# gusanagy/Hybrid-Diffusion-Underwater-Atmopheric-Image-Enhancement

Measured on AMD Instinct MI355X. Metric: denoising-steps/sec (256x256, T=1000), higher is better.
Workload: dtype f32 (tensors and accumulation fp32; every operand of the attention contractions as 2xfp16 pieces -- scores: a balance per product term, four terms at d_head 16 / three at d_head 32; P.V: three terms -- and of the 3x3 convs behind GroupNorm likewise (other 3x3 convs: 3xbf16 pieces), on the 16-bit MFM

## Files before the change

### hybrid-diffusion-underwater-atmopheric-image-enhancement_amd/csrc/attention_x3p.hip

```cpp
#include <stdlib.h>

#include "common.h"
#include "device.h"

using namespace hdiff;

namespace {

constexpr int D = 32;
constexpr int KT = 64;
constexpr int THREADS = 256;
constexpr int NQT = 3;

__global__ __launch_bounds__(THREADS, 2) void mha_flash_fwd_x3p_kernel(const __bf16* __restrict__ ws, float* __restrict__ out,
                                                                      float* __restrict__ lse2, int C, int L, float one) {
  constexpr int KS = D / 16;
  constexpr int KROWB = D * 2 + 16;
  constexpr int KPART = KT * KROWB;
  constexpr int VROWB = KT * 2 + 8;
  constexpr int VPART = D * VROWB;
  constexpr int NKC = NQT * KT * D / 8;
  constexpr int NVC = 2 * D * 8;
  constexpr int NLD = (NKC + NVC) / THREADS;
  static_assert((NKC + NVC) % THREADS == 0, "staging geometry");
  constexpr int QB = 256;
  constexpr int VBASE = NQT * KPART;
  constexpr int BUFB = (VBASE + 2 * VPART + 15) / 16 * 16;
  __shared__ __attribute__((aligned(16))) unsigned char smem[2][BUFB];

  const int tid = threadIdx.x, lane = tid & 63, wave = tid >> 6;
  const int l31 = lane & 31, h = lane >> 5;
  const TileId tile = xcd_tile();
  const int head = tile.head, b = tile.b;
  const int heads = gridDim.y;
  const int qblk0 = tile.x * QB + wave * 64;
  const size_t piece = (size_t)L * D;
  const __bf16* qs = ws + ((size_t)b * heads + head) * F_COUNT * piece;
  const __bf16* ks = qs + F_K * piece;
  const __bf16* vs = qs + F_V * piece;
  const int ntiles = L / KT;

  u32x4 qop[2][NQT][KS];
#pragma unroll
  for (int G = 0; G < 2; ++G) {
    const int q = qblk0 + 32 * G + l31;
#pragma unroll
    for (int p = 0; p < 2; ++p)
#pragma unroll
      for (int s = 0; s < KS; ++s)
        qop[G][p][s] = *reinterpret_cast<const u32x4*>(qs + p * piece + (size_t)q * D + 16 * s + 8 * h);
    const unsigned dn2 = PAIR_DOWN2;
#pragma unroll
    for (int s = 0; s < KS; ++s) {
      unsigned w4[4];
#pragma unroll
      for (int w = 0; w < 4; ++w) asm("v_pk_mul_f16 %0, %1, %2" : "=v"(w4[w]) : "v"(qop[G][0][s][w]), "v"(dn2));
      qop[G][2][s] = u32x4{w4[0], w4[1], w4[2], w4[3]};
    }
  }

  const unsigned char* gsrc[NLD];
  int lds_off[NLD];
  int gstep[NLD];
#pragma unroll
  for (int i = 0; i < NLD; ++i) {
    const int c = i * THREADS + tid;
    if (c < NKC) {
      const int p = c / (KT * D / 8), rem = c - p * (KT * D / 8);
      const int key = rem / (D / 8), part = rem - key * (D / 8);
      gsrc[i] = reinterpret_cast<const unsigned char*>(ks + p * piece) + (size_t)rem * 16;
      lds_off[i] = p * KPART + key * KROWB + part * 16;
      gstep[i] = KT * D * 2;
    } else {
      const int cv = c - NKC;
      const int p = cv / (D * 8), rem = cv - p * (D * 8);
      const int d = rem >> 3, seg = rem & 7;
      gsrc[i] = reinterpret_cast<const unsigned char*>(vs + p * piece + (size_t)d * L) + seg * 16;
      lds_off[i] = VBASE + p * VPART + d * VROWB + seg * 16;
      gstep[i] = KT * 2;
    }
  }
  u32x4 stage[NLD];
  auto stage_load = [&](int t) {
#pragma unroll
    for (int i = 0; i < NLD; ++i) stage[i] = *reinterpret_cast<const u32x4*>(gsrc[i] + (size_t)t * gstep[i]);
  };
  auto stage_store = [&](int buf) {
#pragma unroll
    for (int i = 0; i < NLD; ++i) {
      unsigned char* dst = &smem[buf][lds_off[i]];
      *reinterpret_cast<u32x2*>(dst) = u32x2{stage[i][0], stage[i][1]};
      *reinterpret_cast<u32x2*>(dst + 8) = u32x2{stage[i][2], stage[i][3]};
    }
  };

  const int kaddr = l31 * KROWB + 16 * h;
  int vaddr[2];
#pragma unroll
  for (int p = 0; p < 2; ++p) vaddr[p] = p * VPART + l31 * VROWB + 8 * h;

  f32x16 O[2], negm16;
  f32x2 l_run[2];
  float negm2[2] = {0.f, 0.f};
#pragma unroll
  for (int G = 0; G < 2; ++G) {
    l_run[G] = f32x2{0.f, 0.f};
#pragma unroll
    for (int r = 0; r < 16; ++r) O[G][r] = 0.f;
  }
#pragma unroll
  for (int r = 0; r < 16; ++r) negm16[r] = 0.f;

  auto load_k = [&](int buf, int kb, u32x4 (&kop)[NQT][KS]) {
    const unsigned char* kbuf = smem[buf] + kb * 32 * KROWB + kaddr;
#pragma unroll
    for (int p = 0; p < NQT; ++p)
#pragma unroll
      for (int s = 0; s < KS; ++s) kop[p][s] = *reinterpret_cast<const u32x4*>(kbuf + p * KPART + 32 * s);
  };
  auto load_v = [&](int buf, int kb, u32x4 (&vop)[2][2]) {
    const unsigned char* vbuf = smem[buf] + VBASE + kb * 64;
#pragma unroll
    for (int ab = 0; ab < 2; ++ab)
#pragma unroll
      for (int p = 0; p < 2; ++p) {
        const unsigned char* src = vbuf + vaddr[p] + 32 * ab;
        const u32x2 lo = *reinterpret_cast<const u32x2*>(src);
        const u32x2 hi2 = *reinterpret_cast<const u32x2*>(src + 16);
        vop[ab][p] = u32x4{lo[0], lo[1], hi2[0], hi2[1]};
      }
  };
  auto qk = [&](const u32x4 (&kop)[NQT][KS], int G, f32x16 c) {
    f32x16 S = c;
#pragma unroll
    for (int term = 0; term < NQT; ++term)
#pragma unroll
      for (int s = 0; s < KS; ++s) {
        u32x4 qb = qop[G][term][s];
        if ((HDIFF_MUTANT & 2) && term == 1)
#pragma unroll
          for (int w = 0; w < 4; ++w) qb[w] &= 0xffe0ffe0u;
        S = mfma_f16(kop[term][s], qb, S);
      }
    return S;
  };
  auto exp_pairs = [&](const f32x16& S, u32x4 (&pop)[2][2], float& sum0, float& sum1) {
    sum0 = 0.f; sum1 = 0.f;
#pragma unroll
    for (int j = 0; j < 4; ++j) {
      const float p0 = __builtin_amdgcn_exp2f(S[4 * j]), p1 = __builtin_amdgcn_exp2f(S[4 * j + 1]);
      const float p2 = __builtin_amdgcn_exp2f(S[4 * j + 2]), p3 = __builtin_amdgcn_exp2f(S[4 * j + 3]);
      sum0 += p0 + p2;
      sum1 += p1 + p3;
      unsigned a0, a1, c0, c1;
      split2(p0, p1, one, a0, a1);
      split2(p2, p3, one, c0, c1);
      const int ab = j >> 1, o = (j & 1) * 2;
      pop[ab][0][o] = a0; pop[ab][1][o] = a1;
      pop[ab][0][o + 1] = c0; pop[ab][1][o + 1] = c1;
    }
  };
  auto softmax_pairs = [&](f32x16& S, int G, u32x4 (&pop)[2][2]) {
    float sum0, sum1;
    exp_pairs(S, pop, sum0, sum1);
    if (__builtin_amdgcn_ballot_w64(sum0 + sum1 >= P_TRIP) != 0ull) {
      float mx = fmaxf(fmaxf(S[0], S[1]), fmaxf(S[2], S[3]));
#pragma unroll
      for (int j = 1; j < 4; ++j) mx = fmaxf(mx, fmaxf(fmaxf(S[4 * j], S[4 * j + 1]), fmaxf(S[4 * j + 2], S[4 * j + 3])));
      mx = fmaxf(mx, __shfl_xor(mx, 32, 64));
      const float delta = (mx > P_SHIFT + 1.0f) ? __builtin_ceilf(mx - P_SHIFT) : 0.f;
      const int e = -(int)delta;
#pragma unroll
      for (int r = 0; r < 16; ++r) O[G][r] = __builtin_ldexpf(O[G][r], e);
      l_run[G][0] = __builtin_ldexpf(l_run[G][0], e);
      l_run[G][1] = __builtin_ldexpf(l_run[G][1], e);
      negm2[G] -= delta;
#pragma unroll
      for (int r = 0; r < 16; ++r) S[r] -= delta;
      exp_pairs(S, pop, sum0, sum1);
    }
    l_run[G][0] += sum0;
    l_run[G][1] += sum1;
  };
  auto pv = [&](const u32x4 (&vop)[2][2], const u32x4 (&pop)[2][2], int G) {
#pragma unroll
    for (int ab = 0; ab < 2; ++ab) {
      O[G] = mfma_f16(vop[ab][1], pop[ab][0], O[G]);
      O[G] = mfma_f16(vop[ab][0], pop[ab][1], O[G]);
      O[G] = mfma_f16(vop[ab][0], pop[ab][0], O[G]);
    }
  };

  stage_load(0);
  stage_store(0);
  __syncthreads();
  stage_load(ntiles > 1 ? 1 : 0);
  {
    u32x4 K0[NQT][KS];
    load_k(0, 0, K0);
    const f32x16 s0 = qk(K0, 0, negm16), s1 = qk(K0, 1, negm16);
    float t0 = s0[0], t1 = s1[0];
#pragma unroll
    for (int r = 1; r < 16; ++r) { t0 = fmaxf(t0, s0[r]); t1 = fmaxf(t1, s1[r]); }
    negm2[0] = P_SHIFT - fmaxf(t0, __shfl_xor(t0, 32, 64));
    negm2[1] = P_SHIFT - fmaxf(t1, __shfl_xor(t1, 32, 64));
  }
  auto block = [&](int buf, int kb) {
    u32x4 kop[NQT][KS], vop[2][2];
    load_k(buf, kb, kop);
    load_v(buf, kb, vop);
    f32x16 S2[2];
#pragma unroll
    for (int G = 0; G < 2; ++G) {
      float nm = negm2[G];
      asm volatile("" : "+v"(nm));
#pragma unroll
      for (int r = 0; r < 16; ++r) negm16[r] = nm;
      S2[G] = qk(kop, G, negm16);
    }
#pragma unroll
    for (int G = 0; G < 2; ++G) {
      u32x4 pop[2][2];
      softmax_pairs(S2[G], G, pop);
      pv(vop, pop, G);
    }
  };
  block(0, 0);
  block(0, 1);
  stage_store(1);
  __syncthreads();
  for (int t = 1; t < ntiles; ++t) {
    const int buf = t & 1;
    stage_load((t + 1 < ntiles) ? t + 1 : t);
    block(buf, 0);
    block(buf, 1);
    stage_store(buf ^ 1);
    __syncthreads();
  }

  float* obase = out + ((size_t)b * C + (size_t)head * D) * L;
  const float* vinv = reinterpret_cast<const float*>(qs + 8 * piece);
#pragma unroll
  for (int G = 0; G < 2; ++G) {
    float lt = l_run[G][0] + l_run[G][1];
    lt += __shfl_xor(lt, 32, 64);
    const bool bad = !(lt < OVERFLOW_LIMIT);
    const float inv = bad ? __builtin_nanf("") : 1.0f / lt;
    const int q = qblk0 + 32 * G + l31;
    if (lse2 != nullptr && h == 0)
      lse2[((size_t)b * heads + head) * L + q] = bad ? __builtin_nanf("") : __builtin_amdgcn_logf(lt) - negm2[G];
#pragma unroll
    for (int r = 0; r < 16; ++r) {
      const int d = 8 * (r >> 2) + 4 * h + (r & 3);
      obase[(size_t)d * L + q] = (O[G][r] * inv) * vinv[d];
    }
  }
}

}

namespace hdiff {

int64_t mha_fwd_x3p_workspace(int B, int C, int heads, int L) {
  const int Dh = C / heads;
  if ((Dh != 16 && Dh != 32) || L % 256 != 0 || L < 512) return 0;
  return (int64_t)B * C * L * F_COUNT * 2 + mha_fwd_h2_tail_bytes(B, C);
}

void launch_mha_fwd_x3p(const float* qkv, float* o, float* lse2, int B, int C, int heads, int L, float qscale, void* ws,
                        hipStream_t stream) {
  launch_qk_split_h2(qkv, ws, B, C, heads, L, qscale, stream);
  launch_v_split_h2(qkv, ws, B, C, heads, L, stream);
  hipLaunchKernelGGL(mha_flash_fwd_x3p_kernel, dim3(L / 256, heads, B), dim3(THREADS), 0, stream, (const __bf16*)ws, o, lse2, C, L, 1.0f);
}

}
```

Baseline: 3.045.

## Move rare softmax rescale into out-of-line asm subsection and keep per-group negm vectors

The rarely taken online-softmax rescale path (max reduction, O/l rescale, re-exponentiation) moves into inline-asm blocks placed in a cold subsection behind a scalar branch, so the hot path stays straight-line and the compiler does not keep registers live for it. The running max offset is now held as two persistent 16-wide accumulator-init vectors that are pinned to fixed VGPR ranges, so they no longer need to be broadcast before each QK MFMA. A sched_barrier also separates successive blocks. The hand-written asm and hard-coded register tuples (v[0:15], v[32:47]) are fragile and can clash with the compiler's register allocation. It also relies on manually inserted s_nop hazard padding.

```diff
diff --git a/hybrid-diffusion-underwater-atmopheric-image-enhancement_amd/csrc/attention_x3p.hip b/hybrid-diffusion-underwater-atmopheric-image-enhancement_amd/csrc/attention_x3p.hip
--- a/hybrid-diffusion-underwater-atmopheric-image-enhancement_amd/csrc/attention_x3p.hip
+++ b/hybrid-diffusion-underwater-atmopheric-image-enhancement_amd/csrc/attention_x3p.hip
@@ -11,6 +11,128 @@
 constexpr int KT = 64;
 constexpr int THREADS = 256;
 constexpr int NQT = 3;
+
+#define X3P_RARE_BEGIN "s_cmp_lg_u64 %[cond], 0\n\ts_cbranch_scc1 .Lx3pr_%=\n.Lx3pb_%=:\n\t.subsection 1\n.Lx3pr_%=:\n\t"
+#define X3P_RARE_END "s_branch .Lx3pb_%=\n\t.subsection 0"
+
+__device__ __forceinline__ float x3p_rare_delta(unsigned long long cond, const f32x16& S, int bp32) {
+  float delta, t, u;
+  asm volatile(X3P_RARE_BEGIN
+               "v_max3_f32 %[t], %[s0], %[s1], %[s2]\n\t"
+               "v_max3_f32 %[u], %[s3], %[s4], %[s5]\n\t"
+               "v_max3_f32 %[t], %[t], %[s6], %[s7]\n\t"
+               "v_max3_f32 %[u], %[u], %[s8], %[s9]\n\t"
+               "v_max3_f32 %[t], %[t], %[s10], %[s11]\n\t"
+               "v_max3_f32 %[u], %[u], %[s12], %[s13]\n\t"
+               "v_max3_f32 %[t], %[t], %[s14], %[s15]\n\t"
+               "v_max_f32 %[t], %[t], %[u]\n\t"
+               "s_nop 1\n\t"
+               "ds_bpermute_b32 %[u], %[bp32], %[t]\n\t"
+               "s_waitcnt lgkmcnt(0)\n\t"
+               "v_max_f32 %[t], %[t], %[u]\n\t"
+               "v_subrev_f32 %[u], 8.0, %[t]\n\t"
+               "v_ceil_f32 %[u], %[u]\n\t"
+               "v_cmp_lt_f32 vcc, 0x41100000, %[t]\n\t"
+               "v_cndmask_b32 %[d], 0, %[u], vcc\n\t"
+               X3P_RARE_END
+               : [d] "=&v"(delta), [t] "=&v"(t), [u] "=&v"(u)
+               : [cond] "s"(cond), [bp32] "v"(bp32), [s0] "v"(S[0]), [s1] "v"(S[1]), [s2] "v"(S[2]), [s3] "v"(S[3]), [s4] "v"(S[4]),
+                 [s5] "v"(S[5]), [s6] "v"(S[6]), [s7] "v"(S[7]), [s8] "v"(S[8]), [s9] "v"(S[9]), [s10] "v"(S[10]), [s11] "v"(S[11]),
+                 [s12] "v"(S[12]), [s13] "v"(S[13]), [s14] "v"(S[14]), [s15] "v"(S[15])
+               : "vcc", "scc");
+  return delta;
+}
+
+#define X3P_TIED16(x) [x##0] "+v"(x[0]), [x##1] "+v"(x[1]), [x##2] "+v"(x[2]), [x##3] "+v"(x[3]), [x##4] "+v"(x[4]), [x##5] "+v"(x[5]), \
+                      [x##6] "+v"(x[6]), [x##7] "+v"(x[7]), [x##8] "+v"(x[8]), [x##9] "+v"(x[9]), [x##10] "+v"(x[10]),                  \
+                      [x##11] "+v"(x[11]), [x##12] "+v"(x[12]), [x##13] "+v"(x[13]), [x##14] "+v"(x[14]), [x##15] "+v"(x[15])
+#define X3P_EACH16(op, x, y) op " %[" x "0], %[" x "0], %[" y "]\n\t" op " %[" x "1], %[" x "1], %[" y "]\n\t"       \
+                             op " %[" x "2], %[" x "2], %[" y "]\n\t" op " %[" x "3], %[" x "3], %[" y "]\n\t"       \
+                             op " %[" x "4], %[" x "4], %[" y "]\n\t" op " %[" x "5], %[" x "5], %[" y "]\n\t"       \
+                             op " %[" x "6], %[" x "6], %[" y "]\n\t" op " %[" x "7], %[" x "7], %[" y "]\n\t"       \
+                             op " %[" x "8], %[" x "8], %[" y "]\n\t" op " %[" x "9], %[" x "9], %[" y "]\n\t"       \
+                             op " %[" x "10], %[" x "10], %[" y "]\n\t" op " %[" x "11], %[" x "11], %[" y "]\n\t"   \
+                             op " %[" x "12], %[" x "12], %[" y "]\n\t" op " %[" x "13], %[" x "13], %[" y "]\n\t"   \
+                             op " %[" x "14], %[" x "14], %[" y "]\n\t" op " %[" x "15], %[" x "15], %[" y "]\n\t"
+
+__device__ __forceinline__ void x3p_rare_rescale_o(unsigned long long cond, float delta, f32x16& O) {
+  float o[16], w;
+#pragma unroll
+  for (int r = 0; r < 16; ++r) o[r] = O[r];
+  asm volatile(X3P_RARE_BEGIN
+               "v_cvt_i32_f32 %[w], %[d]\n\t"
+               "v_sub_u32 %[w], 0, %[w]\n\t"
+               X3P_EACH16("v_ldexp_f32", "o", "w")
+               "s_nop 1\n\t"
+               X3P_RARE_END
+               : X3P_TIED16(o), [w] "=&v"(w)
+               : [cond] "s"(cond), [d] "v"(delta)
+               : "scc");
+#pragma unroll
+  for (int r = 0; r < 16; ++r) O[r] = o[r];
+}
+
+#define X3P_EACH16_AT(op, b, y) op " v[%[" b "]+0], v[%[" b "]+0], %[" y "]\n\t" op " v[%[" b "]+1], v[%[" b "]+1], %[" y "]\n\t"       \
+                                op " v[%[" b "]+2], v[%[" b "]+2], %[" y "]\n\t" op " v[%[" b "]+3], v[%[" b "]+3], %[" y "]\n\t"       \
+                                op " v[%[" b "]+4], v[%[" b "]+4], %[" y "]\n\t" op " v[%[" b "]+5], v[%[" b "]+5], %[" y "]\n\t"       \
+                                op " v[%[" b "]+6], v[%[" b "]+6], %[" y "]\n\t" op " v[%[" b "]+7], v[%[" b "]+7], %[" y "]\n\t"       \
+                                op " v[%[" b "]+8], v[%[" b "]+8], %[" y "]\n\t" op " v[%[" b "]+9], v[%[" b "]+9], %[" y "]\n\t"       \
+                                op " v[%[" b "]+10], v[%[" b "]+10], %[" y "]\n\t" op " v[%[" b "]+11], v[%[" b "]+11], %[" y "]\n\t"   \
+                                op " v[%[" b "]+12], v[%[" b "]+12], %[" y "]\n\t" op " v[%[" b "]+13], v[%[" b "]+13], %[" y "]\n\t"   \
+                                op " v[%[" b "]+14], v[%[" b "]+14], %[" y "]\n\t" op " v[%[" b "]+15], v[%[" b "]+15], %[" y "]\n\t"
+#define X3P_RESCALE_REF(TUPLE, BASE)                                                                                       \
+  asm volatile(X3P_RARE_BEGIN                                                                                              \
+               "v_cvt_i32_f32 %[w], %[d]\n\t"                                                                              \
+               "v_sub_u32 %[w], 0, %[w]\n\t"                                                                               \
+               "v_ldexp_f32 %[l0], %[l0], %[w]\n\t"                                                                        \
+               "v_ldexp_f32 %[l1], %[l1], %[w]\n\t"                                                                        \
+               X3P_EACH16_AT("v_sub_f32", "b", "d")                                                                        \
+               "v_mov_b32 %[q0], 0\n\t"                                                                                    \
+               "v_mov_b32 %[q1], 0\n\t"                                                                                    \
+               "s_nop 1\n\t"                                                                                               \
+               X3P_RARE_END                                                                                                \
+               : "+{" TUPLE "}"(negm), [l0] "+v"(l0), [l1] "+v"(l1), [q0] "+v"(sum0), [q1] "+v"(sum1), [w] "=&v"(w)        \
+               : [cond] "s"(cond), [d] "v"(delta), [b] "n"(BASE)                                                           \
+               : "scc")
+template <int G>
+__device__ __forceinline__ void x3p_rare_rescale_ref(unsigned long long cond, float delta, f32x16& negm, f32x2& l, float& sum0,
+                                                     float& sum1) {
+  float l0 = l[0], l1 = l[1], w;
+  if constexpr (G == 0) X3P_RESCALE_REF("v[0:15]", 0);
+  else X3P_RESCALE_REF("v[32:47]", 32);
+  l = f32x2{l0, l1};
+}
+
+__device__ __forceinline__ void x3p_rare_exp_split(unsigned long long cond, float delta, float one, float s0, float s1, float s2, float s3,
+                                                   unsigned& a0, unsigned& a1, unsigned& r0, unsigned& r1, float& sum0, float& sum1) {
+  float p0, p1, p2, p3, t0, t1;
+  asm volatile(X3P_RARE_BEGIN
+               "v_sub_f32 %[p0], %[s0], %[d]\n\t"
+               "v_sub_f32 %[p1], %[s1], %[d]\n\t"
+               "v_sub_f32 %[p2], %[s2], %[d]\n\t"
+               "v_sub_f32 %[p3], %[s3], %[d]\n\t"
+               "v_exp_f32 %[p0], %[p0]\n\t"
+               "v_exp_f32 %[p1], %[p1]\n\t"
+               "v_exp_f32 %[p2], %[p2]\n\t"
+               "v_exp_f32 %[p3], %[p3]\n\t"
+               "s_nop 1\n\t"
+               "v_cvt_pk_f16_f32 %[a0], %[p0], %[p1]\n\t"
+               "v_cvt_pk_f16_f32 %[a1], %[p2], %[p3]\n\t"
+               "v_add_f32 %[t0], %[p0], %[p2]\n\t"
+               "v_add_f32 %[t1], %[p1], %[p3]\n\t"
+               "v_fma_mixlo_f16 %[r0], %[p0], %[one], -%[a0] op_sel_hi:[0,0,1]\n\t"
+               "v_fma_mixlo_f16 %[r1], %[p2], %[one], -%[a1] op_sel_hi:[0,0,1]\n\t"
+               "v_add_f32 %[q0], %[q0], %[t0]\n\t"
+               "v_add_f32 %[q1], %[q1], %[t1]\n\t"
+               "v_fma_mixhi_f16 %[r0], %[p1], %[one], -%[a0] op_sel:[0,0,1] op_sel_hi:[0,0,1]\n\t"
+               "v_fma_mixhi_f16 %[r1], %[p3], %[one], -%[a1] op_sel:[0,0,1] op_sel_hi:[0,0,1]\n\t"
+               "s_nop 1\n\t"
+               X3P_RARE_END
+               : [a0] "+v"(a0), [a1] "+v"(a1), [r0] "+v"(r0), [r1] "+v"(r1), [q0] "+v"(sum0), [q1] "+v"(sum1), [p0] "=&v"(p0),
+                 [p1] "=&v"(p1), [p2] "=&v"(p2), [p3] "=&v"(p3), [t0] "=&v"(t0), [t1] "=&v"(t1)
+               : [cond] "s"(cond), [d] "v"(delta), [one] "s"(one), [s0] "v"(s0), [s1] "v"(s1), [s2] "v"(s2), [s3] "v"(s3)
+               : "scc");
+}
 
 __global__ __launch_bounds__(THREADS, 2) void mha_flash_fwd_x3p_kernel(const __bf16* __restrict__ ws, float* __restrict__ out,
                                                                       float* __restrict__ lse2, int C, int L, float one) {
@@ -99,17 +221,15 @@
 #pragma unroll
   for (int p = 0; p < 2; ++p) vaddr[p] = p * VPART + l31 * VROWB + 8 * h;
 
-  f32x16 O[2], negm16;
+  f32x16 O[2], negm16[2];
   f32x2 l_run[2];
-  float negm2[2] = {0.f, 0.f};
+  const int bp32 = (lane ^ 32) * 4;
 #pragma unroll
   for (int G = 0; G < 2; ++G) {
     l_run[G] = f32x2{0.f, 0.f};
 #pragma unroll
-    for (int r = 0; r < 16; ++r) O[G][r] = 0.f;
-  }
-#pragma unroll
-  for (int r = 0; r < 16; ++r) negm16[r] = 0.f;
+    for (int r = 0; r < 16; ++r) { O[G][r] = 0.f; negm16[G][r] = 0.f; }
+  }
 
   auto load_k = [&](int buf, int kb, u32x4 (&kop)[NQT][KS]) {
     const unsigned char* kbuf = smem[buf] + kb * 32 * KROWB + kaddr;
@@ -130,12 +250,13 @@
         vop[ab][p] = u32x4{lo[0], lo[1], hi2[0], hi2[1]};
       }
   };
-  auto qk = [&](const u32x4 (&kop)[NQT][KS], int G, f32x16 c) {
-    f32x16 S = c;
+  auto qk = [&](const u32x4 (&kop)[NQT][KS], int G) {
+    f32x16 S;
+    asm("v_mfma_f32_32x32x16_f16 %0, %1, %2, %3" : "=&v"(S) : "v"(kop[0][0]), "v"(qop[G][0][0]), "v"(negm16[G]));
 #pragma unroll
     for (int term = 0; term < NQT; ++term)
 #pragma unroll
-      for (int s = 0; s < KS; ++s) {
+      for (int s = (term == 0 ? 1 : 0); s < KS; ++s) {
         u32x4 qb = qop[G][term][s];
         if ((HDIFF_MUTANT & 2) && term == 1)
 #pragma unroll
@@ -144,40 +265,32 @@
       }
     return S;
   };
-  auto exp_pairs = [&](const f32x16& S, u32x4 (&pop)[2][2], float& sum0, float& sum1) {
-    sum0 = 0.f; sum1 = 0.f;
+  auto softmax_pairs = [&](const f32x16& S, int G, u32x4 (&pop)[2][2]) {
+    float sum0, sum1;
+    unsigned a[4][2], rs[4][2];
 #pragma unroll
     for (int j = 0; j < 4; ++j) {
       const float p0 = __builtin_amdgcn_exp2f(S[4 * j]), p1 = __builtin_amdgcn_exp2f(S[4 * j + 1]);
       const float p2 = __builtin_amdgcn_exp2f(S[4 * j + 2]), p3 = __builtin_amdgcn_exp2f(S[4 * j + 3]);
-      sum0 += p0 + p2;
-      sum1 += p1 + p3;
-      unsigned a0, a1, c0, c1;
-      split2(p0, p1, one, a0, a1);
-      split2(p2, p3, one, c0, c1);
+      sum0 = (j == 0) ? p0 + p2 : sum0 + (p0 + p2);
+      sum1 = (j == 0) ? p1 + p3 : sum1 + (p1 + p3);
+      split2(p0, p1, one, a[j][0], rs[j][0]);
+      split2(p2, p3, one, a[j][1], rs[j][1]);
+    }
+    const unsigned long long cond = __builtin_amdgcn_ballot_w64(sum0 + sum1 >= P_TRIP);
+    const float delta = x3p_rare_delta(cond, S, bp32);
+    x3p_rare_rescale_o(cond, delta, O[G]);
+    if (G == 0) x3p_rare_rescale_ref<0>(cond, delta, negm16[0], l_run[0], sum0, sum1);
+    else x3p_rare_rescale_ref<1>(cond, delta, negm16[1], l_run[1], sum0, sum1);
+#pragma unroll
+    for (int j = 0; j < 4; ++j)
+      x3p_rare_exp_split(cond, delta, one, S[4 * j], S[4 * j + 1], S[4 * j + 2], S[4 * j + 3], a[j][0], a[j][1], rs[j][0], rs[j][1], sum0,
+                         sum1);
+#pragma unroll
+    for (int j = 0; j < 4; ++j) {
       const int ab = j >> 1, o = (j & 1) * 2;
-      pop[ab][0][o] = a0; pop[ab][1][o] = a1;
-      pop[ab][0][o + 1] = c0; pop[ab][1][o + 1] = c1;
-    }
-  };
-  auto softmax_pairs = [&](f32x16& S, int G, u32x4 (&pop)[2][2]) {
-    float sum0, sum1;
-    exp_pairs(S, pop, sum0, sum1);
-    if (__builtin_amdgcn_ballot_w64(sum0 + sum1 >= P_TRIP) != 0ull) {
-      float mx = fmaxf(fmaxf(S[0], S[1]), fmaxf(S[2], S[3]));
-#pragma unroll
-      for (int j = 1; j < 4; ++j) mx = fmaxf(mx, fmaxf(fmaxf(S[4 * j], S[4 * j + 1]), fmaxf(S[4 * j + 2], S[4 * j + 3])));
-      mx = fmaxf(mx, __shfl_xor(mx, 32, 64));
-      const float delta = (mx > P_SHIFT + 1.0f) ? __builtin_ceilf(mx - P_SHIFT) : 0.f;
-      const int e = -(int)delta;
-#pragma unroll
-      for (int r = 0; r < 16; ++r) O[G][r] = __builtin_ldexpf(O[G][r], e);
-      l_run[G][0] = __builtin_ldexpf(l_run[G][0], e);
-      l_run[G][1] = __builtin_ldexpf(l_run[G][1], e);
-      negm2[G] -= delta;
-#pragma unroll
-      for (int r = 0; r < 16; ++r) S[r] -= delta;
-      exp_pairs(S, pop, sum0, sum1);
+      pop[ab][0][o] = a[j][0]; pop[ab][1][o] = rs[j][0];
+      pop[ab][0][o + 1] = a[j][1]; pop[ab][1][o + 1] = rs[j][1];
     }
     l_run[G][0] += sum0;
     l_run[G][1] += sum1;
@@ -198,12 +311,13 @@
   {
     u32x4 K0[NQT][KS];
     load_k(0, 0, K0);
-    const f32x16 s0 = qk(K0, 0, negm16), s1 = qk(K0, 1, negm16);
+    const f32x16 s0 = qk(K0, 0), s1 = qk(K0, 1);
     float t0 = s0[0], t1 = s1[0];
 #pragma unroll
     for (int r = 1; r < 16; ++r) { t0 = fmaxf(t0, s0[r]); t1 = fmaxf(t1, s1[r]); }
-    negm2[0] = P_SHIFT - fmaxf(t0, __shfl_xor(t0, 32, 64));
-    negm2[1] = P_SHIFT - fmaxf(t1, __shfl_xor(t1, 32, 64));
+    const float nm0 = P_SHIFT - fmaxf(t0, __shfl_xor(t0, 32, 64)), nm1 = P_SHIFT - fmaxf(t1, __shfl_xor(t1, 32, 64));
+#pragma unroll
+    for (int r = 0; r < 16; ++r) { negm16[0][r] = nm0; negm16[1][r] = nm1; }
   }
   auto block = [&](int buf, int kb) {
     u32x4 kop[NQT][KS], vop[2][2];
@@ -211,19 +325,14 @@
     load_v(buf, kb, vop);
     f32x16 S2[2];
 #pragma unroll
-    for (int G = 0; G < 2; ++G) {
-      float nm = negm2[G];
-      asm volatile("" : "+v"(nm));
-#pragma unroll
-      for (int r = 0; r < 16; ++r) negm16[r] = nm;
-      S2[G] = qk(kop, G, negm16);
-    }
+    for (int G = 0; G < 2; ++G) S2[G] = qk(kop, G);
 #pragma unroll
     for (int G = 0; G < 2; ++G) {
       u32x4 pop[2][2];
       softmax_pairs(S2[G], G, pop);
       pv(vop, pop, G);
     }
+    __builtin_amdgcn_sched_barrier(0);
   };
   block(0, 0);
   block(0, 1);
@@ -248,7 +357,7 @@
     const float inv = bad ? __builtin_nanf("") : 1.0f / lt;
     const int q = qblk0 + 32 * G + l31;
     if (lse2 != nullptr && h == 0)
-      lse2[((size_t)b * heads + head) * L + q] = bad ? __builtin_nanf("") : __builtin_amdgcn_logf(lt) - negm2[G];
+      lse2[((size_t)b * heads + head) * L + q] = bad ? __builtin_nanf("") : __builtin_amdgcn_logf(lt) - negm16[G][0];
 #pragma unroll
     for (int r = 0; r < 16; ++r) {
       const int d = 8 * (r >> 2) + 4 * h + (r & 3);
```

New measurement: 3.050 (median of 6 runs). Within noise of the previous version (+0.2%).
